# insitro/FastVim

Measured on AMD Instinct MI355X. Metric: images/sec FastVim-T 224px bs=128/GPU fwd+bwd (+all-reduce +AdamW +EMA), whole job, higher is better.
Workload: dtype bf16; 1 GPU; FastVim-T 224x224 bs=128/GPU bf16 training step, synthetic ImageNet tensors (BASELINE configs[1]); global_batch=128, parallelism=dp1, hip_graph=True, optimizer_in_step=True, final_loss_hex=0x1.779ca20000000p+0

## Files before the change

### fastvim_amd/_lib.py

```python
import ctypes
import os
import threading

import torch

_PKG = os.path.dirname(os.path.abspath(__file__))
LIB_PATH = os.path.join(_PKG, "libfastvim_hip.so")

FV_F32, FV_BF16, FV_F16 = 0, 1, 2
_DTYPES = {torch.float32: FV_F32, torch.bfloat16: FV_BF16, torch.float16: FV_F16}

_lib = None

C_ABI_SYMBOLS = (
    "fv_last_error", "fv_version",
    "fv_selective_scan_fwd", "fv_selective_scan_bwd_workspace", "fv_selective_scan_bwd",
    "fv_causal_conv1d_fwd", "fv_causal_conv1d_bwd", "fv_scan_expand_skip_fwd",
    "fv_mixer_conv_pool_fwd", "fv_mixer_scan_fwd", "fv_mixer_xproj_scan_fwd_ok", "fv_mixer_xproj_scan_fwd", "fv_mixer_combine_fwd",
    "fv_mixer_bwd_blocks", "fv_mixer_combine_bwd", "fv_mixer_scan_bwd_chunks", "fv_mixer_scan_bwd_chunks_b",
    "fv_mixer_scan_bwd_ckpt_floats", "fv_mixer_scan_bwd_partials", "fv_mixer_scan_bwd", "fv_mixer_scan_bwd_dir", "fv_mixer_scan_bwd_ckpt", "fv_mixer_scan_bwd_segments", "fv_mixer_scan_bwd_seg_floats", "fv_mixer_scan_bwd_seg_partials", "fv_mixer_scan_bwd_seg_chunks", "fv_mixer_scan_bwd_seg", "fv_mixer_scan_fwd_ckpt", "fv_mixer_scan_ckpt_floats", "fv_mixer_scan_fwd_segments", "fv_mixer_scan_fwd_seg_floats", "fv_mixer_scan_fwd_seg", "fv_rows_segment_sum", "fv_rows_gather", "fv_mixer_conv_pool_bwd", "fv_mixer_conv_pool_bwd2_ok", "fv_mixer_conv_pool_bwd2", "fv_mixer_scan_bwd_xproj_ok", "fv_mixer_scan_bwd_xproj", "fv_chunk_rows_bf16", "fv_reduce_partials", "fv_reduce_partials_multi",
    "fv_add_norm_blocks", "fv_add_norm_fwd", "fv_add_norm_bwd", "fv_gemm_bf16", "fv_gemm_bf16_tn_grouped", "fv_gemm_bf16_tn_grouped_ld", "fv_mixer_xproj_fwd", "fv_mixer_xproj_bwd_slices", "fv_mixer_xproj_bwd", "fv_mixer_xproj_bwd2", "fv_mixer_xproj_bwd3_ok", "fv_mixer_xproj_bwd3", "fv_adamw_flat", "fv_soft_target_ce",
    "fv_patch_unfold", "fv_gemm_bf16_rowbias", "fv_mean_pool_fwd", "fv_mean_pool_bwd", "fv_droppath_table", "fv_scale_cast",
    "fv_column_sum", "fv_gemm_bf16_addnorm", "fv_gemm_bf16_dgrad_addnorm_blocks", "fv_gemm_bf16_dgrad_addnorm_bwd", "fv_gemm_bf16_dgrad_addnorm_bwd2", "fv_gemm_bf16_addnorm2", "fv_mixer_combine_out_proj_addnorm_ok", "fv_mixer_combine_out_proj_addnorm", "fv_gemm_f32",
    "fv_mixer_conv_pool_bwd_dgrad_ok", "fv_mixer_conv_pool_bwd_dgrad_blocks", "fv_mixer_conv_pool_bwd_dgrad", "fv_transpose_bf16_batched", "fv_gemm_bf16_tn_grouped_wide8",
    "fv_grad_sumsq_blocks", "fv_grad_sumsq_partials", "fv_adamw_flat_groups",
    "fv_pack_weight_frags_batched", "fv_mixer_conv_pool_bwd_dgrad_pk", "fv_mixer_combine_out_proj_addnorm_pk",
    "fv_mix_batch", "fv_patch_unfold_mix", "fv_mixup_target", "fv_label_ce",
    "fv_patch_unfold_chan", "fv_chan_embed_table", "fv_chan_embed_scatter",
    "fv_mixer_plan",
    "fv_bn1d_stats", "fv_bn1d_apply", "fv_bn1d_bwd", "fv_sgd_flat", "fv_lars_partials_per_segment", "fv_lars_sumsq_partials", "fv_lars_flat",
    "fv_tap_ln_blocks", "fv_tap_ln_fwd", "fv_tap_ln_bwd", "fv_ln2d_blocks", "fv_ln2d_fwd", "fv_ln2d_bwd",
)


_tls = threading.local()


class _DeviceGuarded:

    def __init__(self, cdll):
        self._cdll = cdll
# ... 67 lines not shown
```

### fastvim_amd/csrc/convpool_dgrad.hip

```cpp
#include "mixer_common.h"
#include "packed.h"
#include "gemm_tiles.h"

namespace {

constexpr int CD_DI = 384, CD_N = 192, CD_K = 2 * CD_DI, CD_BM = 64, CD_NT = 256, CD_NCH = CD_DI / 128;
constexpr int CD_RSA = CD_DI * 2 + 16;
constexpr int CD_RSB = CD_N * 2 + 16;
#ifndef CD_PDEPTH
#define CD_PDEPTH 4
#endif
#ifndef CD_SB_EVERY
#define CD_SB_EVERY 1
#endif
#ifndef CD_W2_PIPE
#define CD_W2_PIPE 1
#endif
constexpr int CD_PD = CD_PDEPTH;
constexpr int CD_KS = CD_K / 32;
constexpr int CD_ZST = CD_BM * BK * 2;
constexpr int CD_NZ = CD_DI / BK;
constexpr int CD_O_RING = CD_BM * CD_RSA;
constexpr int CD_SLOT = 12 * 128;
constexpr int CD_O_B = (CD_BM * CD_RSB + 255) / 256 * 256, CD_O_S = CD_O_B + 2 * 128 * BK * 2;
constexpr int CD_SMEM = CD_O_S + 4 * 32 * (64 * 2 + 16);
static_assert(CD_O_RING + 3 * CD_ZST <= CD_SMEM && CD_O_RING + 4 * CD_SLOT * 4 <= CD_SMEM, "LDS regions");
static_assert(2 * CD_SMEM <= 160 * 1024, "two workgroups per CU");
#ifndef CD_FORCE_PK
#define CD_FORCE_PK 0
#endif
#ifndef CD_DBG
#define CD_DBG 0
#endif

struct CdParams {
  const void* xz;
  const void* dob;
  const float* dxc;
  const void* dxc2;
  const float *wf, *bf, *wb, *bb, *Df, *Db;
  void* dxz;
  float* part;
  float pool_scale;
  Geo geo;
  int B;
  const bf16_t* Wt;
  long ldwt;
  const float* dres_out;
// ... 12 lines not shown
  int M;
};

__device__ __forceinline__ void cd_dma16(const void* base, uint32_t voff, uint32_t lds_dst) {
  asm volatile("s_mov_b32 m0, %2\n\ts_nop 0\n\tglobal_load_lds_dwordx4 %0, %1" ::"v"(voff), "s"(base), "s"(lds_dst) : "memory");
}

constexpr int cd_younger(int t) {
  constexpr int KX = CD_DI / 32;
  int n = 0;
  for (int q = KX + 2 * (t - 3) + 2; q < KX + 2 * t; q += 2) n += (q + CD_PD < CD_KS ? 6 : 0) + ((q - KX) / 2 + 3 < CD_NZ ? 2 : 0);
  return n;
}
static_assert(cd_younger(3) < 64 && cd_younger(4) < 64 && cd_younger(5) < 64, "vmcnt is a 6-bit counter");

template <int NT, bool X2, bool PK>
__global__ __launch_bounds__(CD_NT, 2) void conv_pool_bwd_dgrad_kernel(CdParams p) {
  extern __shared__ __attribute__((aligned(16))) char smem[];
  typedef PairVec<bf16_t, 1> P;
  const int tid = threadIdx.x, lane = tid & 63;
  const int wv = __builtin_amdgcn_readfirstlane(tid >> 6);
  const Geo g = p.geo;
  const int tiles = (g.rows + 3) / 4;
  const int bimg = blockIdx.x / tiles, i0 = (blockIdx.x - bimg * tiles) * 4;
  const int mimg = bimg * g.L;
  auto tok_of = [&](int rl) {
    const int w = rl >> 4, j = rl & 15;
    return (i0 + w < g.rows && j < g.cols) ? mimg + (i0 + w) * g.s_i + j * g.s_j : -1;
  };
  const int irow = i0 + wv;
  const bool wlive = irow < g.rows;
// ... 284 lines not shown
        ne_g[it][u][k] = p.dres_out ? *reinterpret_cast<const float4*>(p.dres_out + (size_t)rowc * CD_N + (k * 16 + lr) * 4)
                                    : make_float4(0.f, 0.f, 0.f, 0.f);
    }
  __syncthreads();

#pragma unroll
  for (int b = 0; b < 4; ++b)
#pragma unroll
    for (int a = 0; a < 3; ++a) {
      const f32x4 v = acc[a][b];
      uint2 pk = {pack_bf16x2(v[0], v[1]), pack_bf16x2(v[2], v[3])};
      *reinterpret_cast<uint2*>(smem + (b * 16 + (lane & 15)) * CD_RSB + (wv * 48 + a * 16 + (lane >> 4) * 4) * 2) = pk;
    }
  __syncthreads();
  if (CD_DBG == 3) return;
  {
    constexpr int LPR = 16, RPW = 4, RU = 2, RW = CD_BM / 4;
    const float inv_n = 1.f / (float)CD_N;
    float w[3][4], aw[3][4];
#pragma unroll
    for (int k = 0; k < 3; ++k) {
      const float4 t = *reinterpret_cast<const float4*>(p.nw + (k * LPR + lr) * 4);
      w[k][0] = t.x; w[k][1] = t.y; w[k][2] = t.z; w[k][3] = t.w;
#pragma unroll
      for (int e = 0; e < 4; ++e) aw[k][e] = 0.f;
    }
#pragma unroll
    for (int it = 0; it < RW / (RPW * RU); ++it) {
#pragma unroll
      for (int u = 0; u < RU; ++u) {
// ... 42 lines not shown
          for (int e = 0; e < 4; ++e) dr[e] = rstd * (dxh[k][e] - c1 - xh[k][e] * c2) + gg[e];
          if (live) {
            *reinterpret_cast<float4*>(p.dres_in + base + c) = make_float4(dr[0], dr[1], dr[2], dr[3]);
            if (p.row_scale)
#pragma unroll
              for (int e = 0; e < 4; ++e) dr[e] *= sc;
            uint2 pk = {pack_bf16x2(dr[0], dr[1]), pack_bf16x2(dr[2], dr[3])};
            *reinterpret_cast<uint2*>(p.dx + base + c) = pk;
            *reinterpret_cast<uint2*>(smem + rl * CD_RSB + c * 2) = pk;
          } else {
            *reinterpret_cast<uint2*>(smem + rl * CD_RSB + c * 2) = make_uint2(0u, 0u);
          }
        }
      }
    }
    __syncthreads();
    float* s_acc = reinterpret_cast<float*>(smem + CD_BM * CD_RSB);
#pragma unroll
    for (int k = 0; k < 3; ++k)
#pragma unroll
      for (int e = 0; e < 4; ++e) {
        float v = aw[k][e];
        auto r1 = __builtin_amdgcn_permlane16_swap(__float_as_uint(v), __float_as_uint(v), false, false);
        v = __uint_as_float(r1[0]) + __uint_as_float(r1[1]);
        auto r2 = __builtin_amdgcn_permlane32_swap(__float_as_uint(v), __float_as_uint(v), false, false);
        v = __uint_as_float(r2[0]) + __uint_as_float(r2[1]);
        if (gr == 0) s_acc[wv * CD_N + (k * LPR + lr) * 4 + e] = v;
      }
    __syncthreads();
    float* dst = p.pw + (size_t)blockIdx.x * CD_N;
    for (int c = tid; c < CD_N; c += CD_NT) dst[c] = (s_acc[c] + s_acc[CD_N + c]) + (s_acc[2 * CD_N + c] + s_acc[3 * CD_N + c]);
  }
  if (p.W2 && CD_DBG != 4) {
    __syncthreads();
    tile_times_w2_rows<CD_BM, CD_RSB, KS, decltype(tok_of), CD_W2_PIPE != 0>(smem, smem + CD_O_B, smem + CD_O_S, p.W2, p.ldw2, p.N2,
                                                                              p.C2, tok_of, tid);
  }
}

}

extern "C" int fv_mixer_conv_pool_bwd_dgrad_ok(int batch, int rows, int cols, int tokens_per_patch, int d_inner, int d_model,
                                               int pool_max, int dtype) {
  return dtype == FV_BF16 && d_inner == CD_DI && d_model == CD_N && tokens_per_patch == 1 && !pool_max && batch > 0 &&
         rows > 0 && (cols == 14 || cols == 16) &&
         (long)batch * rows * cols * CD_K * 2 < 0x7fffffffL &&
         (long)batch * rows * CD_DI * 8 < 0x7ffff000L;
}

extern "C" int fv_mixer_conv_pool_bwd_dgrad_blocks(int batch, int rows) { return batch * fv_cdiv(rows, 4); }

static int cd_launch(
    bool packed, const void* xz, const void* dskip, const float* dxc, const void* dxc2, const float* conv_w, const float* conv_b,
    const float* conv_w_b, const float* conv_b_b, const float* D, const float* D_b, void* dxz, float* conv_partials, int batch,
    int rows, int cols, int tok_stride_row, int tok_stride_col, float scaling, const void* W_in_t, long ldwt,
    const float* dresidual_out, const float* r, const float* rstd, const float* norm_weight, const float* row_scale,
    int rows_per_scale, void* dx, float* dresidual_in, float* partial_dw, const void* W2, void* C2, int N2, long ldw2,
    fv_stream_t stream) {
  FV_CHECK(xz && dskip && dxc && conv_w && conv_w_b && dxz && conv_partials && W_in_t && r && rstd && norm_weight && dx &&
               dresidual_in && partial_dw, "mixer_conv_pool_bwd_dgrad: null pointer");
  FV_CHECK(fv_mixer_conv_pool_bwd_dgrad_ok(batch, rows, cols, 1, CD_DI, CD_N, 0, FV_BF16),
           "mixer_conv_pool_bwd_dgrad: shape not built (fv_mixer_conv_pool_bwd_dgrad_ok)");
  FV_CHECK((tok_stride_row == cols && tok_stride_col == 1) || (tok_stride_row == 1 && tok_stride_col == rows),
           "mixer_conv_pool_bwd_dgrad: token strides (%d,%d) are neither row-major nor transposed for a %dx%d grid",
           tok_stride_row, tok_stride_col, rows, cols);
  FV_CHECK(((uintptr_t)W_in_t & 15) == 0 && ldwt % 8 == 0 && ldwt >= CD_K, "mixer_conv_pool_bwd_dgrad: transposed weight rows must be 16-byte aligned");
  FV_CHECK(!packed || ldwt == CD_K, "mixer_conv_pool_bwd_dgrad_pk: the packed weight has no row padding (ldwt = %d)", CD_K);
  FV_CHECK(((uintptr_t)r & 15) == 0 && ((uintptr_t)dresidual_in & 15) == 0 && ((uintptr_t)dx & 7) == 0 &&
               ((uintptr_t)norm_weight & 15) == 0 && ((uintptr_t)dresidual_out & 15) == 0 && ((uintptr_t)dxz & 15) == 0,
           "mixer_conv_pool_bwd_dgrad: row operands must be 16-byte aligned");
  FV_CHECK(!row_scale || rows_per_scale > 0, "mixer_conv_pool_bwd_dgrad: rows_per_scale must be positive");
  FV_CHECK(!W2 || (C2 && N2 > 0 && N2 % 128 == 0 && ldw2 % 8 == 0 && ldw2 >= N2 && ((uintptr_t)W2 & 15) == 0 && ((uintptr_t)C2 & 15) == 0),
           "mixer_conv_pool_bwd_dgrad: the second weight must be (192, N2) with N2 a multiple of 128, 16-byte aligned");
  CdParams p{};
  p.xz = xz; p.dob = dskip; p.dxc = dxc; p.dxc2 = dxc2; p.wf = conv_w; p.bf = conv_b; p.wb = conv_w_b; p.bb = conv_b_b;
  p.Df = D; p.Db = D_b; p.dxz = dxz; p.part = conv_partials;
  p.pool_scale = scaling / (float)cols;
  p.geo = make_geo(rows, cols, tok_stride_row, tok_stride_col, 1);
  p.B = batch;
  p.Wt = (const bf16_t*)W_in_t; p.ldwt = ldwt; p.dres_out = dresidual_out; p.r = r; p.rstd = rstd; p.nw = norm_weight;
  p.row_scale = row_scale; p.rows_per_scale = rows_per_scale > 0 ? rows_per_scale : 1; p.dx = (bf16_t*)dx;
  p.dres_in = dresidual_in; p.pw = partial_dw; p.W2 = (const bf16_t*)W2; p.ldw2 = ldw2; p.C2 = (bf16_t*)C2; p.N2 = N2;
  p.M = batch * rows * cols;
  const dim3 grid(batch * fv_cdiv(rows, 4)), block(CD_NT);
#define FV_CD(NTT, XX, PP)                                                                                          \
  do {                                                                                                              \
    static FvOncePerDevice done;                                                                                    \
    if (done.first())                                                                                               \
      (void)hipFuncSetAttribute((const void*)conv_pool_bwd_dgrad_kernel<NTT, XX, PP>, hipFuncAttributeMaxDynamicSharedMemorySize, CD_SMEM); \
    hipLaunchKernelGGL((conv_pool_bwd_dgrad_kernel<NTT, XX, PP>), grid, block, CD_SMEM, (hipStream_t)stream, p);    \
  } while (0)
#define FV_CD2(NTT, XX) do { if (packed || CD_FORCE_PK) FV_CD(NTT, XX, true); else FV_CD(NTT, XX, false); } while (0)
  if (cols == 14) { if (dxc2) FV_CD2(14, true); else FV_CD2(14, false); }
  else { if (dxc2) FV_CD2(16, true); else FV_CD2(16, false); }
#undef FV_CD2
#undef FV_CD
  FV_LAUNCH_CHECK();
  return FV_OK;
}

#define CD_ARGS_DECL                                                                                                          \
  const void *xz, const void *dskip, const float *dxc, const void *dxc2, const float *conv_w, const float *conv_b,            \
      const float *conv_w_b, const float *conv_b_b, const float *D, const float *D_b, void *dxz, float *conv_partials,        \
      int batch, int rows, int cols, int tok_stride_row, int tok_stride_col, float scaling, const void *W_in_t, long ldwt,    \
      const float *dresidual_out, const float *r, const float *rstd, const float *norm_weight, const float *row_scale,        \
      int rows_per_scale, void *dx, float *dresidual_in, float *partial_dw, const void *W2, void *C2, int N2, long ldw2,      \
      fv_stream_t stream
#define CD_ARGS                                                                                                               \
  xz, dskip, dxc, dxc2, conv_w, conv_b, conv_w_b, conv_b_b, D, D_b, dxz, conv_partials, batch, rows, cols, tok_stride_row,    \
      tok_stride_col, scaling, W_in_t, ldwt, dresidual_out, r, rstd, norm_weight, row_scale, rows_per_scale, dx,              \
      dresidual_in, partial_dw, W2, C2, N2, ldw2, stream

extern "C" int fv_mixer_conv_pool_bwd_dgrad(CD_ARGS_DECL) { return cd_launch(false, CD_ARGS); }

extern "C" int fv_mixer_conv_pool_bwd_dgrad_pk(CD_ARGS_DECL) { return cd_launch(true, CD_ARGS); }
```

### fastvim_amd/csrc/glue.hip

```cpp
#include "common.h"

namespace {

typedef uint32_t u32x4 __attribute__((ext_vector_type(4)));
typedef uint32_t u32x2 __attribute__((ext_vector_type(2)));

template <typename T> struct Vec4;
template <> struct Vec4<float> {
  static __device__ __forceinline__ void ld(const float* p, float (&v)[4]) {
    const float4 t = *reinterpret_cast<const float4*>(p);
    v[0] = t.x; v[1] = t.y; v[2] = t.z; v[3] = t.w;
  }
  static __device__ __forceinline__ void st(float* p, const float (&v)[4]) {
    *reinterpret_cast<float4*>(p) = make_float4(v[0], v[1], v[2], v[3]);
  }
};
template <> struct Vec4<bf16_t> {
  static __device__ __forceinline__ void ld(const bf16_t* p, float (&v)[4]) {
    const u32x2 t = *reinterpret_cast<const u32x2*>(p);
    v[0] = __uint_as_float(t.x << 16); v[1] = __uint_as_float(t.x & 0xffff0000u);
    v[2] = __uint_as_float(t.y << 16); v[3] = __uint_as_float(t.y & 0xffff0000u);
  }
  static __device__ __forceinline__ void st(bf16_t* p, const float (&v)[4]) {
    u32x2 t;
// ... 410 lines not shown
}


constexpr int PKW_ROWS = 192;
struct PackJobs {
  const uint4* src[TRJ_MAX];
  uint4* dst[TRJ_MAX];
  int ks_n;
};
__global__ __launch_bounds__(256) void pack_weight_frags_kernel(PackJobs J) {
  const int u = blockIdx.x * 256 + threadIdx.x;
  if (u >= PKW_ROWS * J.ks_n * 4) return;
  const int lane = u & 63, t = u >> 6, nb = t % 3, ks = (t / 3) % J.ks_n, wv = t / (3 * J.ks_n);
  const int row = 48 * wv + 16 * nb + (lane & 15), unit_in_row = 4 * ks + (lane >> 4);
  J.dst[blockIdx.y][u] = J.src[blockIdx.y][row * (J.ks_n * 4) + unit_in_row];
}

int unfold_store_bytes(int gw, int gjc, size_t patch_bytes) {
  int a = gw, b = gjc;
  while (b) { const int t = a % b; a = b; b = t; }
  const size_t unit = (size_t)a * patch_bytes;
  return unit % 16 == 0 ? 16 : unit % 8 == 0 ? 8 : 4;
}

}

extern "C" int fv_patch_unfold(const void* img, int img_dtype, void* out, int out_dtype, int batch, int chans, int height,
                               int width, int ph, int pw, fv_stream_t stream) {
  FV_CHECK(img && out, "patch_unfold: null pointer");
  FV_CHECK(dt_ok(img_dtype) && dt_ok(out_dtype), "patch_unfold: dtypes must be fp32 or bf16");
// ... 229 lines not shown
extern "C" int fv_pack_weight_frags_batched(const void* const* srcs, void* const* dsts, int njobs, int K, fv_stream_t stream) {
  FV_CHECK(srcs && dsts && njobs > 0 && njobs <= TRJ_MAX, "pack_weight_frags_batched: 1..%d jobs", TRJ_MAX);
  FV_CHECK(K == 384 || K == 768, "pack_weight_frags_batched: K = %d is not a built reduction length (384, 768)", K);
  PackJobs J{};
  for (int j = 0; j < njobs; ++j) {
    FV_CHECK(srcs[j] && dsts[j] && srcs[j] != dsts[j], "pack_weight_frags_batched: null or aliased pointer in job %d", j);
    FV_CHECK(((uintptr_t)srcs[j] & 15) == 0 && ((uintptr_t)dsts[j] & 15) == 0, "pack_weight_frags_batched: job %d is not 16-byte aligned", j);
    J.src[j] = (const uint4*)srcs[j];
    J.dst[j] = (uint4*)dsts[j];
  }
  J.ks_n = K / 32;
  hipLaunchKernelGGL(pack_weight_frags_kernel, dim3(fv_cdiv(PKW_ROWS * J.ks_n * 4, 256), njobs), dim3(256), 0, (hipStream_t)stream, J);
  FV_LAUNCH_CHECK();
  return FV_OK;
}
```

### fastvim_amd/flat.py

```python
import ctypes
import os
import re
import warnings

import torch
import torch.distributed as dist

from . import _lib as L
from .layernorm import RMSNorm
from .mamba_simple_faster import Mamba, _GroupedWgrad, _SideStream, flush_wgrads, group_wgrads
from .mixer_ops import defer_reductions, drop_reductions, flush_reductions, pending_reductions

_LAYER_RE = re.compile(r"^((?:.*\.)?[A-Za-z_]*layers\.\d+)\.")

_MIXER_GROUPS = (
    ("conv", ("conv1d.weight", "conv1d_b.weight", "conv1d.bias", "conv1d_b.bias", "D", "D_b")),
    ("scan", ("A_log", "dt_proj.weight", "dt_proj.bias", "A_b_log", "dt_proj_b.weight", "dt_proj_b.bias")),
    ("ln", ("layernorm.weight", "layernorm.bias")),
    ("xproj", ("x_proj.weight", "x_proj_b.weight")),
)


def _drop_derived_shadows(model):
    for p in model.parameters():
        for a in ("_fv_shadow_t", "_fv_shadow_t_version", "_fv_shadow_pk", "_fv_shadow_pk_version"):
            if hasattr(p, a):
                delattr(p, a)
    for mod in model.modules():
        fv = mod.__dict__.get("_fv")
        if isinstance(fv, dict):
            fv.pop("Wx2_shadow_t", None)
            fv.pop("Wx2_t_params", None)


class FlatTrainingState:
    def __init__(self, model, shadow_dtype=torch.bfloat16, process_group=None, comm_dtype=None,
                 chunk_bytes=256 << 20):
        self.group = process_group
        self.comm_dtype = comm_dtype
        self.chunk = max(1, chunk_bytes // 4)
# ... 94 lines not shown
                if tuple(w.shape) == (768, 192) and w.requires_grad and getattr(w, "_fv_shadow", None) is not None:
                    wt = torch.empty(192, 768, device=dev, dtype=shadow_dtype)
                    w._fv_shadow_t = wt
                    w._fv_shadow_t_version = -1
                    self._t_src.append(w._fv_shadow)
                    self._t_dst.append(wt)
                    self._t_params.append(w)
        self._pk_jobs = {768: ([], [], []), 384: ([], [], [])}
        if shadow_dtype == torch.bfloat16 and dev.type == "cuda":
            for w, wt in zip(self._t_params, self._t_dst):
                self._add_packed(768, w, wt)
            for mod in mixers.values():
                w = getattr(getattr(mod, "out_proj", None), "weight", None)
                if w is not None and tuple(w.shape) == (192, 384) and w.requires_grad and getattr(w, "_fv_shadow", None) is not None:
                    self._add_packed(384, w, w._fv_shadow)
        self._pk_dst = self._pk_jobs[768][1] + self._pk_jobs[384][1]
        self._tx_src, self._tx_dst, self._tx_params = [], [], []
        if shadow_dtype == torch.bfloat16 and dev.type == "cuda":
            for mod in mixers.values():
                fv = mod.__dict__.get("_fv", {})
                ws = fv.get("Wx2_shadow")
                if ws is None or ws.dtype != torch.bfloat16:
                    continue
                _, Wd, d_in = ws.shape
                if d_in >= 768 and d_in % 64 == 0 and Wd % 8 == 0:
                    wt = torch.empty(2, d_in, Wd, device=dev, dtype=shadow_dtype)
                    fv["Wx2_shadow_t"] = wt
                    fv["Wx2_t_params"] = (mod.x_proj.weight, mod.x_proj_b.weight)
                    for k in range(2):
                        self._tx_src.append(ws[k])
                        self._tx_dst.append(wt[k])
# ... 48 lines not shown
                          "were discarded -- call finish_backward() (or allreduce_mean_() / optimizer.step()) after "
                          "loss.backward()", RuntimeWarning, stacklevel=2)
        self.grad_flat.zero_()

    def finish_backward(self):
        flush_wgrads()
        flush_reductions()

    def refresh_shadow(self):
        self.shadow_flat.copy_(self.param_flat)
        for p in self._params:
            p._fv_shadow_version = p._version
        self.refresh_transposed()

    def refresh_transposed(self):
        from .mixer_ops import pack_weight_frags, transpose_bf16_batched
        for src, dst, params in ((self._t_src, self._t_dst, self._t_params),
                                 (getattr(self, "_tx_src", []), getattr(self, "_tx_dst", []), getattr(self, "_tx_params", []))):
            if src:
                transpose_bf16_batched(src, dst)
                for p in params:
                    p._fv_shadow_t_version = p._version
        for srcs, dsts, params in getattr(self, "_pk_jobs", {}).values():
            if srcs:
                pack_weight_frags(srcs, dsts)
                for p in params:
                    p._fv_shadow_pk_version = p._version

    @property
    def world_size(self):
        return dist.get_world_size(self.group) if dist.is_initialized() else 1

    def buckets(self, n_buckets, taper=True):
        blocks = [(i, u) for i, u in enumerate(self.unit_ranges) if u[0] is not None]
        if not blocks:
            return [{"bounds": (0, self.grad_flat.numel()), "layers": (0, 0)}]
        first_u, last_u = blocks[0][0], blocks[-1][0]
        nb = len(blocks)
        n_buckets = max(1, min(n_buckets, nb))
        sizes = [u[2] - u[1] for _, u in blocks]
        w = [i + 2 if taper else 1 for i in range(n_buckets)]
        cum = [sum(sizes) * sum(w[:i + 1]) / sum(w) for i in range(n_buckets)]
# ... 357 lines not shown
```

### fastvim_amd/mamba_simple_faster.py

```python
import ctypes
import math

import torch
import torch.nn as nn
import torch.nn.functional as F

from . import _lib as L
from . import mixer_ops as M
from .gemm import gemm_any_bnn, gemm_any_btn, gemm_any_nn, gemm_any_nt, gemm_any_tn, gemm_nn, gemm_nt, gemm_tn


def _shadow(w, cdt):
    sh = getattr(w, "_fv_shadow", None)
    if sh is not None and sh.dtype == cdt:
        if w._version != w._fv_shadow_version:
            with torch.no_grad():
                sh.copy_(w)
            w._fv_shadow_version = w._version
        return sh
    return w.to(cdt)


def _shadow_t(w, cdt):
    wt = getattr(w, "_fv_shadow_t", None)
# ... 4 lines not shown
            w._fv_shadow_t_version = w._version
        return wt
    return _shadow(w, cdt).t().contiguous()


class _PackedWeights:
    enabled = True


def use_packed_weights(on):
    was = _PackedWeights.enabled
    _PackedWeights.enabled = bool(on)
    return was


def _shadow_pk(w, cdt, plain):
    pk = getattr(w, "_fv_shadow_pk", None)
    if pk is None or pk.dtype != cdt or not _PackedWeights.enabled:
        return None
    if w._version != w._fv_shadow_pk_version:
        if not (plain.is_contiguous() and plain.numel() == pk.numel()):
            return None
        with torch.no_grad():
            M.pack_weight_frags([plain], [pk])
        w._fv_shadow_pk_version = w._version
    return pk


def _wx2_shadow_t(fv):
    if fv is None:
        return None
    wt = fv.get("Wx2_shadow_t")
    if wt is None:
        return None
    params = fv["Wx2_t_params"]
    if any(w._version != w._fv_shadow_t_version for w in params):
        with torch.no_grad():
            for k, w in enumerate(params):
                wt[k].copy_(_shadow(w, wt.dtype).t())
                w._fv_shadow_t_version = w._version
# ... 353 lines not shown
            W_in_c = _shadow(ctx.W_in, cdt)
            dg_prev = torch.empty(Mrows, d_prev, device=dev, dtype=cdt) if W2 is not None else None
            rc = lib.fv_gemm_bf16_dgrad_addnorm_bwd2(
                L.ptr(dxz2), L.ptr(W_in_c), L.ptr(gg), L.ptr(r), L.ptr(rstd), L.ptr(w32), L.ptr(row_scale),
                L.i32(ctx.rows_per_scale), L.ptr(dx), L.ptr(dres_in), L.ptr(pw), L.i32(Mrows), L.i32(d),
                L.i32(dxz2.shape[1]), ctypes.c_long(dxz2.stride(0)), ctypes.c_long(d), L.ptr(W2), L.ptr(dg_prev),
                L.i32(d_prev if W2 is not None else 0), ctypes.c_long(d_prev), L.stream_of(dxz2))
            L.check(rc, "gemm_bf16_dgrad_addnorm_bwd")
            out.update(dx=dx, dres_in=dres_in, pw=pw, nb=nb, dg_prev=dg_prev)

        def fused_conv_dgrad(xz, d_o, dxc, dxc2, cw2, cb, cwb2, cb_b, D, D_b, dxz, rows, cols, transposed, scaling, conv_grad_out):
            gg = dres_out.reshape(Mrows, d).contiguous() if dres_out is not None else None
            d_prev = g_prev.shape[2]
            W2 = _shadow(W_out_prev, cdt) if d_prev % 128 == 0 else None
            W_in_t = _shadow_t(ctx.W_in, cdt)
            p2, dx, dres_in, pw, nb, dg_prev = M.conv_pool_bwd_dgrad(
                xz, d_o, dxc, dxc2, cw2, cb, cwb2, cb_b, D, D_b, dxz, rows, cols, transposed, scaling, W_in_t, gg, r, rstd,
                w32, row_scale, ctx.rows_per_scale, W2=W2, conv_grad_out=conv_grad_out, W_in_pk=_shadow_pk(ctx.W_in, cdt, W_in_t))
            out.update(dx=dx, dres_in=dres_in, pw=pw, nb=nb, dg_prev=dg_prev)
            return p2

        fctx.fused_in_dgrad = fused_in_dgrad
        if (CONV_IN_DGRAD and cdt == torch.bfloat16 and d == 192 and ctx.W_in.shape[0] == 768 and (row_scale is None or row_scale.dtype == torch.float32)):
            fctx.fused_conv_dgrad = fused_conv_dgrad
        grads = FastVimMixerFn.backward(fctx, dg)
        with torch.autocast("cuda", enabled=False):
            gd = _direct_grad(ctx.w_param)
            if gd is not None:
                M.reduce_partials(out["pw"], out["nb"], out=gd.view(-1), accumulate=True)
                dw = None
            else:
                dw = M.reduce_partials(out["pw"], out["nb"]).to(ctx.w_param.dtype)
            dx = out["dx"]
# ... 321 lines not shown
```

### fastvim_amd/mixer_ops.py

```python
import ctypes

import torch

from . import _lib as L

f32 = ctypes.c_float


def _geo(rows, cols, transposed):
    return (1, rows) if transposed else (cols, 1)


def conv_pool_fwd(xz, conv_w, conv_b, conv_w_b, conv_b_b, rows, cols, transposed, pool_max, scaling, tpp=1,
                  D=None, D_b=None):
    B, Ltok, two_d = xz.shape
    d_in = two_d // 2
    s_i, s_j = _geo(rows, cols, transposed)
    xc = torch.empty(2, B, rows * tpp, d_in, device=xz.device, dtype=xz.dtype)
    skip = torch.empty(B, Ltok, d_in, device=xz.device, dtype=xz.dtype) if D is not None else None
    amax = torch.empty_like(xc) if pool_max else None
    rc = L.lib().fv_mixer_conv_pool_fwd(
        L.ptr(xz), L.ptr(conv_w), L.ptr(conv_b), L.ptr(conv_w_b), L.ptr(conv_b_b), L.ptr(D), L.ptr(D_b), L.ptr(xc),
        L.ptr(skip), L.ptr(amax), L.i32(B), L.i32(rows), L.i32(cols), L.i32(s_i), L.i32(s_j), L.i32(tpp), L.i32(d_in),
        L.i32(conv_w.shape[-1]), L.i32(pool_max), f32(scaling), L.i32(L.dtype_code(xz.dtype)), L.stream_of(xz))
# ... 302 lines not shown
    if grad_out is not None:
        reduce_partials(part, nb, out=grad_out, accumulate=True)
        return None
    return reduce_partials(part, nb)


def conv_pool_bwd_dgrad_ok(xz, rows, cols, tpp, d_model, pool_max):
    B, Ltok, two_d = xz.shape
    return bool(xz.dtype == torch.bfloat16 and xz.is_contiguous() and
                L.lib().fv_mixer_conv_pool_bwd_dgrad_ok(L.i32(B), L.i32(rows), L.i32(cols), L.i32(tpp), L.i32(two_d // 2),
                                                        L.i32(d_model), L.i32(int(bool(pool_max))), L.i32(L.FV_BF16)))


def conv_pool_bwd_dgrad(xz, d_o, dxc, dxc2, conv_w, conv_b, conv_w_b, conv_b_b, D, D_b, dxz, rows, cols, transposed, scaling,
                        W_in_t, dres_out, r, rstd, norm_w32, row_scale, rows_per_scale, W2=None, conv_grad_out=None,
                        W_in_pk=None):
    B, Ltok, two_d = xz.shape
    d_in = two_d // 2
    d = W_in_t.shape[0]
    Mrows = B * Ltok
    s_i, s_j = _geo(rows, cols, transposed)
    lib = L.lib()
    dev = xz.device
    nb = lib.fv_mixer_conv_pool_bwd_dgrad_blocks(L.i32(B), L.i32(rows))
    part = torch.empty(nb, 12 * d_in, device=dev, dtype=torch.float32)
    dx = torch.empty(Mrows, d, device=dev, dtype=torch.bfloat16)
    dres_in = torch.empty(Mrows, d, device=dev, dtype=torch.float32)
    pw = torch.empty(nb, d, device=dev, dtype=torch.float32)
    N2 = W2.shape[1] if W2 is not None else 0
    dg_prev = torch.empty(Mrows, N2, device=dev, dtype=torch.bfloat16) if W2 is not None else None
    assert dxc2 is None or (dxc2.dtype == xz.dtype and dxc2.shape == dxc.shape and dxc2.is_contiguous())
    assert W_in_t.dtype == torch.bfloat16 and W_in_t.stride(1) == 1 and W_in_t.shape[1] == two_d
    if W_in_pk is not None:
        assert W_in_pk.dtype == torch.bfloat16 and W_in_pk.is_contiguous() and W_in_pk.numel() == d * two_d
        fn, W_arg, ldwt = lib.fv_mixer_conv_pool_bwd_dgrad_pk, W_in_pk, two_d
    else:
        fn, W_arg, ldwt = lib.fv_mixer_conv_pool_bwd_dgrad, W_in_t, W_in_t.stride(0)
    rc = fn(
        L.ptr(xz), L.ptr(d_o), L.ptr(dxc), L.ptr(dxc2), L.ptr(conv_w), L.ptr(conv_b), L.ptr(conv_w_b), L.ptr(conv_b_b),
        L.ptr(D), L.ptr(D_b), L.ptr(dxz), L.ptr(part), L.i32(B), L.i32(rows), L.i32(cols), L.i32(s_i), L.i32(s_j),
        f32(scaling), L.ptr(W_arg), ctypes.c_long(ldwt), L.ptr(dres_out), L.ptr(r), L.ptr(rstd), L.ptr(norm_w32),
        L.ptr(row_scale), L.i32(rows_per_scale), L.ptr(dx), L.ptr(dres_in), L.ptr(pw), L.ptr(W2), L.ptr(dg_prev), L.i32(N2),
        ctypes.c_long(W2.stride(0) if W2 is not None else 0), L.stream_of(xz))
    L.check(rc, "mixer_conv_pool_bwd_dgrad")
    if conv_grad_out is not None:
        reduce_partials(part, nb, out=conv_grad_out, accumulate=True)
        p2 = None
    else:
        p2 = reduce_partials(part, nb)
    return p2, dx, dres_in, pw, nb, dg_prev


def transpose_bf16_batched(srcs, dsts):
    lib = L.lib()
    rows, cols = srcs[0].shape
    for lo in range(0, len(srcs), 64):
        a, b = srcs[lo:lo + 64], dsts[lo:lo + 64]
        assert all(t.dtype == torch.bfloat16 and t.is_contiguous() and tuple(t.shape) == (rows, cols) for t in a)
# ... 24 lines not shown
    return W[idx[:, 0:1], cols].reshape(rows, K)


def pack_weight_frags(srcs, dsts):
    lib = L.lib()
    rows, K = srcs[0].shape
    for lo in range(0, len(srcs), 64):
        a, b = srcs[lo:lo + 64], dsts[lo:lo + 64]
        assert all(t.dtype == torch.bfloat16 and t.is_contiguous() and tuple(t.shape) == (rows, K) for t in a)
        assert all(t.dtype == torch.bfloat16 and t.is_contiguous() and t.numel() == rows * K for t in b)
        assert rows == PACK_ROWS
        k = len(a)
        ins = (ctypes.c_void_p * k)(*[t.data_ptr() for t in a])
        outs = (ctypes.c_void_p * k)(*[t.data_ptr() for t in b])
        L.check(lib.fv_pack_weight_frags_batched(ins, outs, L.i32(k), L.i32(K), L.stream_of(a[0])), "pack_weight_frags_batched")


XPROJ_WIDTHS = (44, 56, 80, 96, 112, 34, 36, 38, 64)


def xproj_fwd(xc, Wx2_c):
    d_in = xc.shape[-1]
    Mrows = xc.numel() // (2 * d_in)
    W = Wx2_c.shape[1]
    if (xc.dtype != torch.bfloat16 or Wx2_c.dtype != torch.bfloat16 or d_in % 32 or W > 112
            or not xc.is_contiguous() or not Wx2_c.is_contiguous() or xc.data_ptr() % 16 or Wx2_c.data_ptr() % 16):
        if xc.is_cuda and xc.dtype in (torch.float32, torch.bfloat16) and Wx2_c.dtype in (torch.float32, torch.bfloat16):
            from .gemm import gemm_any_bnt
            return gemm_any_bnt(xc.reshape(2, Mrows, d_in), Wx2_c)
        return torch.bmm(xc.view(2, Mrows, d_in), Wx2_c.transpose(1, 2))
# ... 75 lines not shown
```

### include/fastvim_hip.h

```cpp
#ifndef FASTVIM_HIP_H
#define FASTVIM_HIP_H

#include <stddef.h>
#include <stdint.h>

#ifdef __cplusplus
extern "C" {
#endif

typedef void* fv_stream_t;

enum { FV_F32 = 0, FV_BF16 = 1, FV_F16 = 2 };
enum { FV_OK = 0, FV_ERR_INVALID = -1, FV_ERR_HIP = -2, FV_ERR_UNSUPPORTED = -3 };

const char* fv_last_error(void);
#define FV_ABI_VERSION 3
int fv_version(void);

int fv_selective_scan_fwd(const void* u, const void* delta, const float* A, const void* B,
                          const void* C, const float* D, const void* z, const float* delta_bias,
                          void* out, float* last_state, int batch, int dim, int seqlen, int dstate,
                          int n_groups, int B_variable, int C_variable, int delta_softplus,
                          int dtype, fv_stream_t stream);

// ... 188 lines not shown
                                 const float* D, const float* D_b, void* dxz, float* conv_partials, int batch, int rows,
                                 int cols, int tok_stride_row, int tok_stride_col, float scaling, const void* W_in_t,
                                 long ldwt, const float* dresidual_out, const float* r, const float* rstd,
                                 const float* norm_weight, const float* row_scale, int rows_per_scale, void* dx,
                                 float* dresidual_in, float* partial_dw, const void* W2, void* C2, int N2, long ldw2,
                                 fv_stream_t stream);
int fv_mixer_conv_pool_bwd_dgrad_pk(const void* xz, const void* dskip, const float* dxc, const void* dxc2,
                                    const float* conv_w, const float* conv_b, const float* conv_w_b,
                                    const float* conv_b_b, const float* D, const float* D_b, void* dxz,
                                    float* conv_partials, int batch, int rows, int cols, int tok_stride_row,
                                    int tok_stride_col, float scaling, const void* W_in_t, long ldwt,
                                    const float* dresidual_out, const float* r, const float* rstd,
                                    const float* norm_weight, const float* row_scale, int rows_per_scale, void* dx,
                                    float* dresidual_in, float* partial_dw, const void* W2, void* C2, int N2, long ldw2,
                                    fv_stream_t stream);

int fv_transpose_bf16_batched(const void* const* srcs, void* const* dsts, int njobs, int rows, int cols,
                              fv_stream_t stream);

int fv_pack_weight_frags_batched(const void* const* srcs, void* const* dsts, int njobs, int K, fv_stream_t stream);

int fv_gemm_bf16_addnorm2(const void* A, const void* W, const float* residual, const float* norm_weight,
                          const float* row_scale, int rows_per_scale, void* y, float* residual_out, float* rstd, int M,
                          int N, int K, long lda, long ldw, float eps, const void* W2, void* C2, int N2, long ldw2,
                          fv_stream_t stream);

int fv_gemm_bf16_tn_grouped(const void* const* x, const void* const* y, float* const* parts, const int* Kd,
                            const int* M, const int* N, const int* splits, int count, fv_stream_t stream);
int fv_gemm_bf16_tn_grouped_ld(const void* const* x, const void* const* y, float* const* parts, const int* Kd,
                               const int* M, const int* N, const int* ldx, const int* ldy, const int* splits, int count,
                               fv_stream_t stream);

int fv_gemm_bf16_tn_grouped_wide8(int M, int N, int Kd);

int fv_mixer_xproj_fwd(const void* xc, const void* x_proj_w2, void* x_dbl, int M, int d_inner, int width,
// ... 87 lines not shown
```

Before: 24900 images/sec.

## Feed second dgrad GEMM from pre-packed MFMA weight fragments held in registers

Adds a packed fragment layout for the 192x384 out_proj weight, a batched pack kernel, and a PK2 variant of the conv-pool dgrad kernel. In this variant each wave loads its W2 fragments straight from global memory into a register ring, prefilled during the tail of the first phase, and no longer stages W2 through LDS in the shared tile_times_w2_rows path. It is meant to remove LDS staging and barriers from the fused second GEMM. In exchange it keeps an extra packed shadow copy per weight, needs repacking whenever the weight changes, and raises register pressure in a kernel whose launch bounds ask for two workgroups per CU.

```diff
diff --git a/fastvim_amd/_lib.py b/fastvim_amd/_lib.py
--- a/fastvim_amd/_lib.py
+++ b/fastvim_amd/_lib.py
@@ -25,6 +25,7 @@
     "fv_mixer_conv_pool_bwd_dgrad_ok", "fv_mixer_conv_pool_bwd_dgrad_blocks", "fv_mixer_conv_pool_bwd_dgrad", "fv_transpose_bf16_batched", "fv_gemm_bf16_tn_grouped_wide8",
     "fv_grad_sumsq_blocks", "fv_grad_sumsq_partials", "fv_adamw_flat_groups",
     "fv_pack_weight_frags_batched", "fv_mixer_conv_pool_bwd_dgrad_pk", "fv_mixer_combine_out_proj_addnorm_pk",
+    "fv_pack_weight_frags_w2_batched", "fv_mixer_conv_pool_bwd_dgrad_pk2",
     "fv_mix_batch", "fv_patch_unfold_mix", "fv_mixup_target", "fv_label_ce",
     "fv_patch_unfold_chan", "fv_chan_embed_table", "fv_chan_embed_scatter",
     "fv_mixer_plan",
diff --git a/fastvim_amd/csrc/convpool_dgrad.hip b/fastvim_amd/csrc/convpool_dgrad.hip
--- a/fastvim_amd/csrc/convpool_dgrad.hip
+++ b/fastvim_amd/csrc/convpool_dgrad.hip
@@ -15,6 +15,12 @@
 #endif
 #ifndef CD_W2_PIPE
 #define CD_W2_PIPE 1
+#endif
+#ifndef CD_W2_PASSES
+#define CD_W2_PASSES 1
+#endif
+#ifndef CD_W2_PDEPTH
+#define CD_W2_PDEPTH 3
 #endif
 constexpr int CD_PD = CD_PDEPTH;
 constexpr int CD_KS = CD_K / 32;
@@ -32,6 +38,13 @@
 #ifndef CD_DBG
 #define CD_DBG 0
 #endif
+constexpr int CD_W2_KS = CD_N / 32, CD_W2_P = CD_W2_PASSES, CD_W2_NBP = 6 / CD_W2_P, CD_W2_STEPS = CD_W2_KS * CD_W2_P;
+constexpr int CD_W2_RING = CD_W2_PDEPTH * CD_W2_P;
+constexpr int CD_W2_RS = CD_W2_NBP * 32 + 16;
+constexpr int CD_W2_ROWS = 16 * CD_W2_P;
+static_assert(CD_W2_P == 1 || CD_W2_P == 2, "one pass of 96 columns or two of 48");
+static_assert(CD_W2_RING >= 1 && CD_W2_RING <= CD_W2_STEPS, "ring depth");
+static_assert(CD_W2_ROWS * CD_W2_RS <= 32 * (64 * 2 + 16), "the wave's slab");
 
 struct CdParams {
   const void* xz;
@@ -74,7 +87,7 @@
 }
 static_assert(cd_younger(3) < 64 && cd_younger(4) < 64 && cd_younger(5) < 64, "vmcnt is a 6-bit counter");
 
-template <int NT, bool X2, bool PK>
+template <int NT, bool X2, bool PK, bool PK2 = false>
 __global__ __launch_bounds__(CD_NT, 2) void conv_pool_bwd_dgrad_kernel(CdParams p) {
   extern __shared__ __attribute__((aligned(16))) char smem[];
   typedef PairVec<bf16_t, 1> P;
@@ -389,6 +402,19 @@
     }
   __syncthreads();
   if (CD_DBG == 3) return;
+  bf16x8 w2f[PK2 ? CD_W2_RING : 1][CD_W2_NBP];
+  const char* w2pk = reinterpret_cast<const char*>(p.W2) + wv * (CD_W2_KS * 6 * 1024);
+  auto w2frag = [&](int a, int s) {
+    return *reinterpret_cast<const bf16x8*>(w2pk + ((s % CD_W2_KS) * 6 + (s / CD_W2_KS) * CD_W2_NBP + a) * 1024 + (uint32_t)lane * 16);
+  };
+  auto w2prefill = [&]() {
+    __builtin_amdgcn_sched_barrier(0);
+#pragma unroll
+    for (int s = 0; s < CD_W2_RING; ++s)
+#pragma unroll
+      for (int a = 0; a < CD_W2_NBP; ++a) w2f[s][a] = w2frag(a, s);
+    __builtin_amdgcn_sched_barrier(0);
+  };
   {
     constexpr int LPR = 16, RPW = 4, RU = 2, RW = CD_BM / 4;
     const float inv_n = 1.f / (float)CD_N;
@@ -461,6 +487,7 @@
         }
       }
     }
+    if constexpr (PK2 && CD_DBG != 4) w2prefill();
     __syncthreads();
     float* s_acc = reinterpret_cast<float*>(smem + CD_BM * CD_RSB);
 #pragma unroll
@@ -478,7 +505,60 @@
     float* dst = p.pw + (size_t)blockIdx.x * CD_N;
     for (int c = tid; c < CD_N; c += CD_NT) dst[c] = (s_acc[c] + s_acc[CD_N + c]) + (s_acc[2 * CD_N + c] + s_acc[3 * CD_N + c]);
   }
-  if (p.W2 && CD_DBG != 4) {
+  if constexpr (PK2) {
+    if (CD_DBG == 4) return;
+    char* my = smem + CD_O_S + wv * (32 * (64 * 2 + 16));
+    const char* afrag = smem + (lane & 15) * CD_RSB + (lane >> 4) * 16;
+    f32x4 acc[CD_W2_NBP][4];
+    static_for<CD_W2_STEPS>([&](auto s_c) {
+      constexpr int s = decltype(s_c)::value, ks = s % CD_W2_KS, pass = s / CD_W2_KS;
+      if constexpr (ks == 0) {
+#pragma unroll
+        for (int a = 0; a < CD_W2_NBP; ++a)
+#pragma unroll
+          for (int b = 0; b < 4; ++b) acc[a][b] = (f32x4){0.f, 0.f, 0.f, 0.f};
+      }
+      bf16x8 cur[CD_W2_NBP];
+#pragma unroll
+      for (int a = 0; a < CD_W2_NBP; ++a) cur[a] = w2f[s % CD_W2_RING][a];
+      if constexpr (s + CD_W2_RING < CD_W2_STEPS) {
+#pragma unroll
+        for (int a = 0; a < CD_W2_NBP; ++a) w2f[s % CD_W2_RING][a] = w2frag(a, s + CD_W2_RING);
+      }
+      __builtin_amdgcn_sched_barrier(0);
+      bf16x8 fa[4];
+#pragma unroll
+      for (int b = 0; b < 4; ++b) fa[b] = *reinterpret_cast<const bf16x8*>(afrag + b * 16 * CD_RSB + ks * 64);
+#pragma unroll
+      for (int a = 0; a < CD_W2_NBP; ++a)
+#pragma unroll
+        for (int b = 0; b < 4; ++b) acc[a][b] = __builtin_amdgcn_mfma_f32_16x16x32_bf16(cur[a], fa[b], acc[a][b], 0, 0, 0);
+      __builtin_amdgcn_sched_barrier(0);
+      if constexpr (ks == CD_W2_KS - 1) {
+        constexpr int CH = CD_W2_NBP * 2;
+#pragma unroll
+        for (int h = 0; h < 64 / CD_W2_ROWS; ++h) {
+#pragma unroll
+          for (int bb = 0; bb < CD_W2_P; ++bb)
+#pragma unroll
+            for (int a = 0; a < CD_W2_NBP; ++a) {
+              const f32x4 v = acc[a][h * CD_W2_P + bb];
+              uint2 pk = {pack_bf16x2(v[0], v[1]), pack_bf16x2(v[2], v[3])};
+              *reinterpret_cast<uint2*>(my + (bb * 16 + (lane & 15)) * CD_W2_RS + (a * 16 + (lane >> 4) * 4) * 2) = pk;
+            }
+          __builtin_amdgcn_wave_barrier();
+#pragma unroll
+          for (int i = 0; i < CD_W2_ROWS * CH / 64; ++i) {
+            const int idx = i * 64 + lane, r = idx / CH, ch = idx - r * CH;
+            const int m = tok_of(h * CD_W2_ROWS + r), n = wv * 96 + pass * (CD_W2_NBP * 16) + ch * 8;
+            if (CD_DBG == 5 ? m == -2 : m >= 0)
+              *reinterpret_cast<u32x4*>(p.C2 + (long)m * CD_DI + n) = *reinterpret_cast<const u32x4*>(my + r * CD_W2_RS + ch * 16);
+          }
+          __builtin_amdgcn_wave_barrier();
+        }
+      }
+    });
+  } else if (p.W2 && CD_DBG != 4) {
     __syncthreads();
     tile_times_w2_rows<CD_BM, CD_RSB, KS, decltype(tok_of), CD_W2_PIPE != 0>(smem, smem + CD_O_B, smem + CD_O_S, p.W2, p.ldw2, p.N2,
                                                                               p.C2, tok_of, tid);
@@ -498,7 +578,7 @@
 extern "C" int fv_mixer_conv_pool_bwd_dgrad_blocks(int batch, int rows) { return batch * fv_cdiv(rows, 4); }
 
 static int cd_launch(
-    bool packed, const void* xz, const void* dskip, const float* dxc, const void* dxc2, const float* conv_w, const float* conv_b,
+    int packed, const void* xz, const void* dskip, const float* dxc, const void* dxc2, const float* conv_w, const float* conv_b,
     const float* conv_w_b, const float* conv_b_b, const float* D, const float* D_b, void* dxz, float* conv_partials, int batch,
     int rows, int cols, int tok_stride_row, int tok_stride_col, float scaling, const void* W_in_t, long ldwt,
     const float* dresidual_out, const float* r, const float* rstd, const float* norm_weight, const float* row_scale,
@@ -517,6 +597,8 @@
                ((uintptr_t)norm_weight & 15) == 0 && ((uintptr_t)dresidual_out & 15) == 0 && ((uintptr_t)dxz & 15) == 0,
            "mixer_conv_pool_bwd_dgrad: row operands must be 16-byte aligned");
   FV_CHECK(!row_scale || rows_per_scale > 0, "mixer_conv_pool_bwd_dgrad: rows_per_scale must be positive");
+  FV_CHECK(packed != 2 || (W2 && C2 && N2 == CD_DI && ldw2 == CD_DI),
+           "mixer_conv_pool_bwd_dgrad_pk2: the packed second weight is (192, %d) without row padding, and not null", CD_DI);
   FV_CHECK(!W2 || (C2 && N2 > 0 && N2 % 128 == 0 && ldw2 % 8 == 0 && ldw2 >= N2 && ((uintptr_t)W2 & 15) == 0 && ((uintptr_t)C2 & 15) == 0),
            "mixer_conv_pool_bwd_dgrad: the second weight must be (192, N2) with N2 a multiple of 128, 16-byte aligned");
   CdParams p{};
@@ -530,14 +612,19 @@
   p.dres_in = dresidual_in; p.pw = partial_dw; p.W2 = (const bf16_t*)W2; p.ldw2 = ldw2; p.C2 = (bf16_t*)C2; p.N2 = N2;
   p.M = batch * rows * cols;
   const dim3 grid(batch * fv_cdiv(rows, 4)), block(CD_NT);
-#define FV_CD(NTT, XX, PP)                                                                                          \
+#define FV_CD(NTT, XX, PP, P2)                                                                                      \
   do {                                                                                                              \
     static FvOncePerDevice done;                                                                                    \
     if (done.first())                                                                                               \
-      (void)hipFuncSetAttribute((const void*)conv_pool_bwd_dgrad_kernel<NTT, XX, PP>, hipFuncAttributeMaxDynamicSharedMemorySize, CD_SMEM); \
-    hipLaunchKernelGGL((conv_pool_bwd_dgrad_kernel<NTT, XX, PP>), grid, block, CD_SMEM, (hipStream_t)stream, p);    \
+      (void)hipFuncSetAttribute((const void*)conv_pool_bwd_dgrad_kernel<NTT, XX, PP, P2>, hipFuncAttributeMaxDynamicSharedMemorySize, CD_SMEM); \
+    hipLaunchKernelGGL((conv_pool_bwd_dgrad_kernel<NTT, XX, PP, P2>), grid, block, CD_SMEM, (hipStream_t)stream, p); \
   } while (0)
-#define FV_CD2(NTT, XX) do { if (packed || CD_FORCE_PK) FV_CD(NTT, XX, true); else FV_CD(NTT, XX, false); } while (0)
+#define FV_CD2(NTT, XX)                                              \
+  do {                                                               \
+    if (packed == 2) FV_CD(NTT, XX, true, true);                     \
+    else if (packed || CD_FORCE_PK) FV_CD(NTT, XX, true, false);     \
+    else FV_CD(NTT, XX, false, false);                               \
+  } while (0)
   if (cols == 14) { if (dxc2) FV_CD2(14, true); else FV_CD2(14, false); }
   else { if (dxc2) FV_CD2(16, true); else FV_CD2(16, false); }
 #undef FV_CD2
@@ -558,6 +645,8 @@
       tok_stride_col, scaling, W_in_t, ldwt, dresidual_out, r, rstd, norm_weight, row_scale, rows_per_scale, dx,              \
       dresidual_in, partial_dw, W2, C2, N2, ldw2, stream
 
-extern "C" int fv_mixer_conv_pool_bwd_dgrad(CD_ARGS_DECL) { return cd_launch(false, CD_ARGS); }
-
-extern "C" int fv_mixer_conv_pool_bwd_dgrad_pk(CD_ARGS_DECL) { return cd_launch(true, CD_ARGS); }
+extern "C" int fv_mixer_conv_pool_bwd_dgrad(CD_ARGS_DECL) { return cd_launch(0, CD_ARGS); }
+
+extern "C" int fv_mixer_conv_pool_bwd_dgrad_pk(CD_ARGS_DECL) { return cd_launch(1, CD_ARGS); }
+
+extern "C" int fv_mixer_conv_pool_bwd_dgrad_pk2(CD_ARGS_DECL) { return cd_launch(2, CD_ARGS); }
diff --git a/fastvim_amd/csrc/glue.hip b/fastvim_amd/csrc/glue.hip
--- a/fastvim_amd/csrc/glue.hip
+++ b/fastvim_amd/csrc/glue.hip
@@ -448,6 +448,22 @@
   const int lane = u & 63, t = u >> 6, nb = t % 3, ks = (t / 3) % J.ks_n, wv = t / (3 * J.ks_n);
   const int row = 48 * wv + 16 * nb + (lane & 15), unit_in_row = 4 * ks + (lane >> 4);
   J.dst[blockIdx.y][u] = J.src[blockIdx.y][row * (J.ks_n * 4) + unit_in_row];
+}
+
+constexpr int PKW2_N = 384, PKW2_UNITS = PKW_ROWS * PKW2_N / 8;
+struct PackJobsW2 {
+  const uint16_t* src[TRJ_MAX];
+  uint4* dst[TRJ_MAX];
+};
+__global__ __launch_bounds__(256) void pack_weight_frags_w2_kernel(PackJobsW2 J) {
+  const int u = blockIdx.x * 256 + threadIdx.x;
+  if (u >= PKW2_UNITS) return;
+  const int lane = u & 63, t = u >> 6, nb = t % 6, ks = (t / 6) % 6, wv = t / 36;
+  const uint16_t* s = J.src[blockIdx.y] + (32 * ks + 8 * (lane >> 4)) * PKW2_N + 96 * wv + 16 * nb + (lane & 15);
+  uint32_t w[4];
+#pragma unroll
+  for (int j = 0; j < 4; ++j) w[j] = (uint32_t)s[(2 * j) * PKW2_N] | ((uint32_t)s[(2 * j + 1) * PKW2_N] << 16);
+  J.dst[blockIdx.y][u] = make_uint4(w[0], w[1], w[2], w[3]);
 }
 
 int unfold_store_bytes(int gw, int gjc, size_t patch_bytes) {
@@ -707,3 +723,17 @@
   FV_LAUNCH_CHECK();
   return FV_OK;
 }
+
+extern "C" int fv_pack_weight_frags_w2_batched(const void* const* srcs, void* const* dsts, int njobs, fv_stream_t stream) {
+  FV_CHECK(srcs && dsts && njobs > 0 && njobs <= TRJ_MAX, "pack_weight_frags_w2_batched: 1..%d jobs", TRJ_MAX);
+  PackJobsW2 J{};
+  for (int j = 0; j < njobs; ++j) {
+    FV_CHECK(srcs[j] && dsts[j] && srcs[j] != dsts[j], "pack_weight_frags_w2_batched: null or aliased pointer in job %d", j);
+    FV_CHECK(((uintptr_t)srcs[j] & 1) == 0 && ((uintptr_t)dsts[j] & 15) == 0, "pack_weight_frags_w2_batched: job %d is not aligned", j);
+    J.src[j] = (const uint16_t*)srcs[j];
+    J.dst[j] = (uint4*)dsts[j];
+  }
+  hipLaunchKernelGGL(pack_weight_frags_w2_kernel, dim3(fv_cdiv(PKW2_UNITS, 256), njobs), dim3(256), 0, (hipStream_t)stream, J);
+  FV_LAUNCH_CHECK();
+  return FV_OK;
+}
diff --git a/fastvim_amd/flat.py b/fastvim_amd/flat.py
--- a/fastvim_amd/flat.py
+++ b/fastvim_amd/flat.py
@@ -23,7 +23,8 @@
 
 def _drop_derived_shadows(model):
     for p in model.parameters():
-        for a in ("_fv_shadow_t", "_fv_shadow_t_version", "_fv_shadow_pk", "_fv_shadow_pk_version"):
+        for a in ("_fv_shadow_t", "_fv_shadow_t_version", "_fv_shadow_pk", "_fv_shadow_pk_version",
+                  "_fv_shadow_pk2", "_fv_shadow_pk2_version"):
             if hasattr(p, a):
                 delattr(p, a)
     for mod in model.modules():
@@ -148,7 +149,15 @@
                 w = getattr(getattr(mod, "out_proj", None), "weight", None)
                 if w is not None and tuple(w.shape) == (192, 384) and w.requires_grad and getattr(w, "_fv_shadow", None) is not None:
                     self._add_packed(384, w, w._fv_shadow)
-        self._pk_dst = self._pk_jobs[768][1] + self._pk_jobs[384][1]
+        self._pk2_src, self._pk2_dst, self._pk2_params = [], [], []
+        for w, src in zip(self._pk_jobs[384][2], self._pk_jobs[384][0]):
+            pk2 = torch.empty(192 * 384, device=dev, dtype=shadow_dtype)
+            w._fv_shadow_pk2 = pk2
+            w._fv_shadow_pk2_version = -1
+            self._pk2_src.append(src)
+            self._pk2_dst.append(pk2)
+            self._pk2_params.append(w)
+        self._pk_dst = self._pk_jobs[768][1] + self._pk_jobs[384][1] + self._pk2_dst
         self._tx_src, self._tx_dst, self._tx_params = [], [], []
         if shadow_dtype == torch.bfloat16 and dev.type == "cuda":
             for mod in mixers.values():
@@ -227,7 +236,7 @@
         self.refresh_transposed()
 
     def refresh_transposed(self):
-        from .mixer_ops import pack_weight_frags, transpose_bf16_batched
+        from .mixer_ops import pack_weight_frags, pack_weight_frags_w2, transpose_bf16_batched
         for src, dst, params in ((self._t_src, self._t_dst, self._t_params),
                                  (getattr(self, "_tx_src", []), getattr(self, "_tx_dst", []), getattr(self, "_tx_params", []))):
             if src:
@@ -239,6 +248,10 @@
                 pack_weight_frags(srcs, dsts)
                 for p in params:
                     p._fv_shadow_pk_version = p._version
+        if getattr(self, "_pk2_src", []):
+            pack_weight_frags_w2(self._pk2_src, self._pk2_dst)
+            for p in self._pk2_params:
+                p._fv_shadow_pk2_version = p._version
 
     @property
     def world_size(self):
diff --git a/fastvim_amd/mamba_simple_faster.py b/fastvim_amd/mamba_simple_faster.py
--- a/fastvim_amd/mamba_simple_faster.py
+++ b/fastvim_amd/mamba_simple_faster.py
@@ -42,16 +42,16 @@
     return was
 
 
-def _shadow_pk(w, cdt, plain):
-    pk = getattr(w, "_fv_shadow_pk", None)
+def _shadow_pk(w, cdt, plain, attr="_fv_shadow_pk", pack=None):
+    pk = getattr(w, attr, None)
     if pk is None or pk.dtype != cdt or not _PackedWeights.enabled:
         return None
-    if w._version != w._fv_shadow_pk_version:
+    if w._version != getattr(w, attr + "_version"):
         if not (plain.is_contiguous() and plain.numel() == pk.numel()):
             return None
         with torch.no_grad():
-            M.pack_weight_frags([plain], [pk])
-        w._fv_shadow_pk_version = w._version
+            (pack or M.pack_weight_frags)([plain], [pk])
+        setattr(w, attr + "_version", w._version)
     return pk
 
 
@@ -435,9 +435,12 @@
             d_prev = g_prev.shape[2]
             W2 = _shadow(W_out_prev, cdt) if d_prev % 128 == 0 else None
             W_in_t = _shadow_t(ctx.W_in, cdt)
+            W_in_pk = _shadow_pk(ctx.W_in, cdt, W_in_t)
+            W2_pk = (_shadow_pk(W_out_prev, cdt, W2, "_fv_shadow_pk2", M.pack_weight_frags_w2)
+                     if W2 is not None and W_in_pk is not None else None)
             p2, dx, dres_in, pw, nb, dg_prev = M.conv_pool_bwd_dgrad(
                 xz, d_o, dxc, dxc2, cw2, cb, cwb2, cb_b, D, D_b, dxz, rows, cols, transposed, scaling, W_in_t, gg, r, rstd,
-                w32, row_scale, ctx.rows_per_scale, W2=W2, conv_grad_out=conv_grad_out, W_in_pk=_shadow_pk(ctx.W_in, cdt, W_in_t))
+                w32, row_scale, ctx.rows_per_scale, W2=W2, conv_grad_out=conv_grad_out, W_in_pk=W_in_pk, W2_pk=W2_pk)
             out.update(dx=dx, dres_in=dres_in, pw=pw, nb=nb, dg_prev=dg_prev)
             return p2
 
diff --git a/fastvim_amd/mixer_ops.py b/fastvim_amd/mixer_ops.py
--- a/fastvim_amd/mixer_ops.py
+++ b/fastvim_amd/mixer_ops.py
@@ -340,7 +340,7 @@
 
 def conv_pool_bwd_dgrad(xz, d_o, dxc, dxc2, conv_w, conv_b, conv_w_b, conv_b_b, D, D_b, dxz, rows, cols, transposed, scaling,
                         W_in_t, dres_out, r, rstd, norm_w32, row_scale, rows_per_scale, W2=None, conv_grad_out=None,
-                        W_in_pk=None):
+                        W_in_pk=None, W2_pk=None):
     B, Ltok, two_d = xz.shape
     d_in = two_d // 2
     d = W_in_t.shape[0]
@@ -355,19 +355,24 @@
     pw = torch.empty(nb, d, device=dev, dtype=torch.float32)
     N2 = W2.shape[1] if W2 is not None else 0
     dg_prev = torch.empty(Mrows, N2, device=dev, dtype=torch.bfloat16) if W2 is not None else None
+    W2_arg, ldw2 = W2, (W2.stride(0) if W2 is not None else 0)
     assert dxc2 is None or (dxc2.dtype == xz.dtype and dxc2.shape == dxc.shape and dxc2.is_contiguous())
     assert W_in_t.dtype == torch.bfloat16 and W_in_t.stride(1) == 1 and W_in_t.shape[1] == two_d
     if W_in_pk is not None:
         assert W_in_pk.dtype == torch.bfloat16 and W_in_pk.is_contiguous() and W_in_pk.numel() == d * two_d
         fn, W_arg, ldwt = lib.fv_mixer_conv_pool_bwd_dgrad_pk, W_in_pk, two_d
+        if W2_pk is not None and W2 is not None:
+            assert tuple(W2.shape) == (PACK_ROWS, PACK_W2_N) and W2_pk.dtype == torch.bfloat16 and W2_pk.is_contiguous()
+            assert W2_pk.numel() == W2.numel()
+            fn, W2_arg, ldw2 = lib.fv_mixer_conv_pool_bwd_dgrad_pk2, W2_pk, PACK_W2_N
     else:
         fn, W_arg, ldwt = lib.fv_mixer_conv_pool_bwd_dgrad, W_in_t, W_in_t.stride(0)
     rc = fn(
         L.ptr(xz), L.ptr(d_o), L.ptr(dxc), L.ptr(dxc2), L.ptr(conv_w), L.ptr(conv_b), L.ptr(conv_w_b), L.ptr(conv_b_b),
         L.ptr(D), L.ptr(D_b), L.ptr(dxz), L.ptr(part), L.i32(B), L.i32(rows), L.i32(cols), L.i32(s_i), L.i32(s_j),
         f32(scaling), L.ptr(W_arg), ctypes.c_long(ldwt), L.ptr(dres_out), L.ptr(r), L.ptr(rstd), L.ptr(norm_w32),
-        L.ptr(row_scale), L.i32(rows_per_scale), L.ptr(dx), L.ptr(dres_in), L.ptr(pw), L.ptr(W2), L.ptr(dg_prev), L.i32(N2),
-        ctypes.c_long(W2.stride(0) if W2 is not None else 0), L.stream_of(xz))
+        L.ptr(row_scale), L.i32(rows_per_scale), L.ptr(dx), L.ptr(dres_in), L.ptr(pw), L.ptr(W2_arg), L.ptr(dg_prev), L.i32(N2),
+        ctypes.c_long(ldw2), L.stream_of(xz))
     L.check(rc, "mixer_conv_pool_bwd_dgrad")
     if conv_grad_out is not None:
         reduce_partials(part, nb, out=conv_grad_out, accumulate=True)
@@ -422,6 +427,36 @@
         ins = (ctypes.c_void_p * k)(*[t.data_ptr() for t in a])
         outs = (ctypes.c_void_p * k)(*[t.data_ptr() for t in b])
         L.check(lib.fv_pack_weight_frags_batched(ins, outs, L.i32(k), L.i32(K), L.stream_of(a[0])), "pack_weight_frags_batched")
+
+
+PACK_W2_N = 384
+
+
+def pack_index_w2():
+    u = torch.arange(PACK_ROWS * PACK_W2_N // 8)
+    lane, t = u % 64, u // 64
+    nb, ks, wv = t % 6, (t // 6) % 6, t // 36
+    row = (32 * ks + 8 * (lane // 16))[:, None] + torch.arange(8)
+    col = (96 * wv + 16 * nb + (lane % 16))[:, None].expand(-1, 8)
+    return torch.stack([row, col], dim=2)
+
+
+def pack_weight_frags_w2_ref(W):
+    assert tuple(W.shape) == (PACK_ROWS, PACK_W2_N)
+    idx = pack_index_w2().to(W.device)
+    return W[idx[..., 0], idx[..., 1]].reshape(PACK_ROWS, PACK_W2_N)
+
+
+def pack_weight_frags_w2(srcs, dsts):
+    lib = L.lib()
+    for lo in range(0, len(srcs), 64):
+        a, b = srcs[lo:lo + 64], dsts[lo:lo + 64]
+        assert all(t.dtype == torch.bfloat16 and t.is_contiguous() and tuple(t.shape) == (PACK_ROWS, PACK_W2_N) for t in a)
+        assert all(t.dtype == torch.bfloat16 and t.is_contiguous() and t.numel() == PACK_ROWS * PACK_W2_N for t in b)
+        k = len(a)
+        ins = (ctypes.c_void_p * k)(*[t.data_ptr() for t in a])
+        outs = (ctypes.c_void_p * k)(*[t.data_ptr() for t in b])
+        L.check(lib.fv_pack_weight_frags_w2_batched(ins, outs, L.i32(k), L.stream_of(a[0])), "pack_weight_frags_w2_batched")
 
 
 XPROJ_WIDTHS = (44, 56, 80, 96, 112, 34, 36, 38, 64)
diff --git a/include/fastvim_hip.h b/include/fastvim_hip.h
--- a/include/fastvim_hip.h
+++ b/include/fastvim_hip.h
@@ -226,11 +226,22 @@
                                     const float* norm_weight, const float* row_scale, int rows_per_scale, void* dx,
                                     float* dresidual_in, float* partial_dw, const void* W2, void* C2, int N2, long ldw2,
                                     fv_stream_t stream);
+int fv_mixer_conv_pool_bwd_dgrad_pk2(const void* xz, const void* dskip, const float* dxc, const void* dxc2,
+                                     const float* conv_w, const float* conv_b, const float* conv_w_b,
+                                     const float* conv_b_b, const float* D, const float* D_b, void* dxz,
+                                     float* conv_partials, int batch, int rows, int cols, int tok_stride_row,
+                                     int tok_stride_col, float scaling, const void* W_in_t, long ldwt,
+                                     const float* dresidual_out, const float* r, const float* rstd,
+                                     const float* norm_weight, const float* row_scale, int rows_per_scale, void* dx,
+                                     float* dresidual_in, float* partial_dw, const void* W2, void* C2, int N2, long ldw2,
+                                     fv_stream_t stream);
 
 int fv_transpose_bf16_batched(const void* const* srcs, void* const* dsts, int njobs, int rows, int cols,
                               fv_stream_t stream);
 
 int fv_pack_weight_frags_batched(const void* const* srcs, void* const* dsts, int njobs, int K, fv_stream_t stream);
+
+int fv_pack_weight_frags_w2_batched(const void* const* srcs, void* const* dsts, int njobs, fv_stream_t stream);
 
 int fv_gemm_bf16_addnorm2(const void* A, const void* W, const float* residual, const float* norm_weight,
                           const float* row_scale, int rows_per_scale, void* y, float* residual_out, float* rstd, int M,
```

Measured after the change: 25160 images/sec (median of 6 runs). +1.0%, better.
